# zhaoruiyang98/eftpipe

Measured on AMD Instinct MI355X. Metric: theory P_l(k) evaluations/sec (single tracer, Nk=512, l=0,2,4), higher is better.
Workload: dtype f64

## Files before the change

### eftpipe_amd/csrc/eftb_kernels.hpp

```cpp
#pragma once
#include <hip/hip_runtime.h>
#include <stdint.h>
#include <stdlib.h>

namespace eftb {

constexpr int NS = 80;
constexpr int NPOW = 257;
constexpr int NHALF = 128;
constexpr int NCH = 129;

constexpr int NROW = 24;

typedef double v4d __attribute__((ext_vector_type(4)));
typedef double v2d __attribute__((ext_vector_type(2)));

__device__ __forceinline__ void xcd_decode(int ntile, int& tile, int& group) {
    const int flat = blockIdx.x, ng = gridDim.x / ntile;
    if ((ng & 7) == 0) {
        const int slot = flat >> 3;
        tile = slot % ntile;
        group = (flat & 7) + 8 * (slot / ntile);
    } else {
        tile = flat % ntile;
// ... 1650 lines not shown
    double h[2];
#pragma unroll
    for (int v = 0; v < 2; ++v) h[v] = H[((size_t)v * NS + s0) * Nk + kc];
    double z = k2 * ct[42], y = k2 * ct[43];
    double b0, b1;
    powers(z * (1.0 / RS_ZS), b0, b1);
#pragma unroll
    for (int tau = 0; tau < NT; ++tau)
#pragma unroll
        for (int t = 0; t < 2; ++t) asm volatile("" : "+v"(aop[tau][t]));
    for (int s = s0; s < s1; ++s) {
        const int sn = s + 1 < s1 ? s + 1 : s;
        const double* ctn = RSC + ((size_t)w * NS + sn) * RS_REC;
        double cv[14 * NT];
#pragma unroll
        for (int i = 0; i < 14 * NT; ++i) cv[i] = ct[i];
        const double xn = ctn[42], yn0 = ctn[43];
        double hn[2];
#pragma unroll
        for (int v = 0; v < 2; ++v) hn[v] = H[((size_t)v * NS + sn) * Nk + kc];
        __builtin_amdgcn_sched_barrier(0);
        v4d D[NT];
#pragma unroll
        for (int tau = 0; tau < NT; ++tau) D[tau] = __builtin_amdgcn_mfma_f64_16x16x4f64(aop[tau][0], b0, (v4d){0.0, 0.0, 0.0, 0.0}, 0, 0, 0);
#pragma unroll
        for (int tau = 0; tau < NT; ++tau) D[tau] = __builtin_amdgcn_mfma_f64_16x16x4f64(aop[tau][1], b1, D[tau], 0, 0, 0);
        __builtin_amdgcn_sched_barrier(0);
        const double zn = k2 * xn, yn = k2 * yn0;
        double bn0, bn1;
        powers(zn * (1.0 / RS_ZS), bn0, bn1);
        const double zh[2] = {z * h[0], z * h[1]}, yh[2] = {y * h[0], y * h[1]};
#pragma unroll
        for (int tau = 0; tau < NT; ++tau) {
            const double W = fma(zh[tau], D[tau][0], fma(yh[0], D[tau][1], yh[1] * D[tau][2]));
            acc11[tau] = fma(W, cv[tau * 14], acc11[tau]);
            accCt[tau] = fma(W, cv[tau * 14 + 1], accCt[tau]);
#pragma unroll
            for (int i = 0; i < 12; ++i) accL[i] = fma(W, cv[tau * 14 + 2 + i], accL[i]);
        }
        __builtin_amdgcn_sched_barrier(0);
        ct = ctn;
        z = zn;
        y = yn;
        b0 = bn0;
        b1 = bn1;
        h[0] = hn[0];
        h[1] = hn[1];
    }
    if (!live) return;
    const int l = jg & 1;
    double o18[18], oA[3];
#pragma unroll
    for (int i = 0; i < 6; ++i) o18[i] = lct[i] * accCt[0] + lct[6 + i] * accCt[1];
#pragma unroll
    for (int i = 0; i < 12; ++i) o18[6 + i] = accL[i];
#pragma unroll
    for (int i = 0; i < 3; ++i) oA[i] = l11[i] * acc11[0] + l11[3 + i] * acc11[1];
    if (nsplit == 1) {
        double* dst = T + (((size_t)w * NL + l) * NROW) * Nk + k;
        if (jg < 2) {
#pragma unroll
            for (int i = 0; i < 18; ++i) dst[(size_t)(3 + i) * Nk] += o18[i];
        } else {
#pragma unroll
            for (int i = 0; i < 3; ++i) dst[(size_t)i * Nk] += oA[i];
        }
    } else {
        double* pw = part + (((size_t)w * nsplit + split) * NL + l) * 21 * Nk + k;
        if (jg < 2) {
#pragma unroll
            for (int i = 0; i < 18; ++i) pw[(size_t)(3 + i) * Nk] = o18[i];
        } else {
#pragma unroll
            for (int i = 0; i < 3; ++i) pw[(size_t)i * Nk] = oA[i];
        }
    }
}

__global__ __launch_bounds__(256) void resum_sum_kernel(int Nk, int Nl, int nchunk, const double* __restrict__ part,
                                                        double* __restrict__ T) {
    const int k = blockIdx.x * blockDim.x + threadIdx.x;
    const int i = blockIdx.y % 21, l = blockIdx.y / 21, w = blockIdx.z;
    if (k >= Nk) return;
    double a = 0.0;
    for (int c = 0; c < nchunk; ++c) a += part[((((size_t)w * nchunk + c) * Nl + l) * 21 + i) * Nk + k];
    T[(((size_t)w * Nl + l) * NROW + i) * Nk + k] += a;
}

constexpr int SPL_HB = 32;

constexpr int SPL_W = 128, SPL_LD = SPL_W + 2;

__global__ __launch_bounds__(256) __attribute__((amdgpu_num_vgpr(88))) void spline_kernel(int Nk, int nseries, int rlo, int rsel, const double* __restrict__ T, const double* __restrict__ band,
                                                     double* __restrict__ S) {
    __shared__ double ys[16 * SPL_LD];
    const int tid = threadIdx.x, lane = tid & 63, wave = tid >> 6, r = lane & 15, g = lane >> 4;
    int ktile, share;
    xcd_decode((Nk + 63) / 64, ktile, share);
    const int nshare = gridDim.x / ((Nk + 63) / 64);
    const int w0 = ktile * 64 - SPL_HB;
    const int it0 = ktile * 64 + 16 * wave;
    double bf[20];
#pragma unroll
    for (int t = 0; t < 20; ++t) {
        const int d = 4 * t + g - r, i = it0 + r;
        bf[t] = (d >= 0 && d <= 2 * SPL_HB && i < Nk) ? band[(size_t)d * Nk + i] : 0.0;
    }
    const int ngroups = (nseries + 15) / 16;
    const int per = (ngroups + nshare - 1) / nshare;
    const int g0 = share * per, g1 = min(ngroups, g0 + per);
    auto row_of = [&](int sp) { return rsel == NROW ? sp : (sp / rsel) * NROW + rlo + sp % rsel; };
    double pre[8];
    auto fetch = [&](int grp) {
#pragma unroll
        for (int u = 0; u < 8; ++u) {
            const int e = tid + 256 * u, sr = e >> 7, jj = w0 + (e & 127), series = grp * 16 + sr;
            pre[u] = (series < nseries && jj >= 0 && jj < Nk) ? T[(size_t)row_of(series) * Nk + jj] : 0.0;
        }
    };
    if (g0 < g1) fetch(g0);
    for (int grp = g0; grp < g1; ++grp) {
        __syncthreads();
#pragma unroll
        for (int u = 0; u < 8; ++u) {
            const int e = tid + 256 * u;
            ys[(e >> 7) * SPL_LD + (e & 127)] = pre[u];
        }
        __syncthreads();
        if (grp + 1 < g1) fetch(grp + 1);
        v4d acc = (v4d){0.0, 0.0, 0.0, 0.0};
        const double* yr = ys + r * SPL_LD + 16 * wave + g;
#pragma unroll
        for (int t = 0; t < 20; ++t) acc = __builtin_amdgcn_mfma_f64_16x16x4f64(yr[4 * t], bf[t], acc, 0, 0, 0);
        const int i = it0 + r;
#pragma unroll
        for (int q = 0; q < 4; ++q) {
            const int sr = g + 4 * q, series = grp * 16 + sr;
            if (series < nseries && i < Nk) S[(size_t)row_of(series) * Nk + i] = acc[q];
        }
    }
}

__device__ __forceinline__ int bspl_first(int i, int Nk) { return min(max(i - 1, 0), Nk - 4); }

__device__ inline int knot_interval(const double* __restrict__ kk, int Nk, double x) {
    int lo = 0, hi = Nk - 1;
    while (hi - lo > 1) {
        const int mid = (lo + hi) >> 1;
        if (kk[mid] <= x) lo = mid; else hi = mid;
    }
    return lo;
}

template <int NL>
__global__ __launch_bounds__(320) void ap_prefix_kernel(int nmu, const double* __restrict__ DAw, const double* __restrict__ Hw,
                                                        const double* __restrict__ fid, const double* __restrict__ mu,
                                                        const double* __restrict__ wmu, const double* __restrict__ legmu,
                                                        double* __restrict__ PS, double* __restrict__ ROOT) {
    constexpr int NS = NL * NL * 4, NCH = 8;
    extern __shared__ double sm[];
    double* s_rho = sm;
    double* s_lp = sm + nmu;
    double* s_wl = sm + (1 + NL) * nmu;
    double* s_tot = sm + (1 + 2 * NL) * nmu;
    const int w = blockIdx.x;
    const double qperp = DAw[w] / fid[0], qpar = fid[1] / Hw[w];
    const double F = qpar / qperp, g = 1.0 / (F * F) - 1.0;
    for (int j = threadIdx.x; j < nmu; j += blockDim.x) {
        const double m = mu[j];
        const double root = sqrt(1.0 + m * m * g);
        const double mp = m / (F * root), x2 = mp * mp;
        ROOT[(size_t)w * nmu + j] = root;
        s_rho[j] = g * m * m / (1.0 + root);
        s_lp[j] = 1.0;
        s_lp[nmu + j] = 0.5 * (3.0 * x2 - 1.0);
        if (NL > 2) s_lp[2 * nmu + j] = (35.0 * x2 * x2 - 30.0 * x2 + 3.0) * 0.125;
#pragma unroll
        for (int l = 0; l < NL; ++l) s_wl[l * nmu + j] = wmu[j] * legmu[l * nmu + j];
    }
    __syncthreads();
    const int seq = threadIdx.x % NS, ch = threadIdx.x / NS;
    const int q = seq & 3, l = (seq >> 2) % NL, lp = seq / (4 * NL);
    const int clen = (nmu + NCH - 1) / NCH, j0 = ch * clen, j1 = min(nmu, j0 + clen);
    double* ps = PS + (size_t)w * (nmu + 1) * NS + seq;
    auto term = [&](int j) {
        const double r = s_rho[j];
        const double rq = q == 0 ? 1.0 : (q == 1 ? r : (q == 2 ? r * r : r * r * r));
        return s_wl[l * nmu + j] * s_lp[lp * nmu + j] * rq;
    };
    if (ch < NCH) {
        double s = 0.0;
        for (int j = j0; j < j1; ++j) s += term(j);
        s_tot[seq * NCH + ch] = s;
    }
    __syncthreads();
    if (threadIdx.x < NS) {
        double run = 0.0;
        for (int c = 0; c < NCH; ++c) {
            const double t = s_tot[threadIdx.x * NCH + c];
            s_tot[threadIdx.x * NCH + c] = run;
            run += t;
        }
        PS[(size_t)w * (nmu + 1) * NS + threadIdx.x] = 0.0;
    }
    __syncthreads();
    if (ch < NCH) {
        double s = s_tot[seq * NCH + ch];
        for (int j = j0; j < j1; ++j) {
            s += term(j);
            ps[(size_t)(j + 1) * NS] = s;
        }
    }
}

template <int NL, bool BSPL>
__global__ __launch_bounds__(64) void ap_direct_kernel(int Nk, int nmu, int rlo, int nr, const double* __restrict__ kk, const double* __restrict__ DAw,
                                                       const double* __restrict__ Hw, const double* __restrict__ fid,
                                                       const double* __restrict__ mu, const double* __restrict__ wmu,
                                                       const double* __restrict__ legmu, const double* __restrict__ ROOT,
                                                       const double* __restrict__ T, const double* __restrict__ S, double* __restrict__ Tout,
                                                       const int4* __restrict__ META, const double* __restrict__ bias, double* __restrict__ Plk,
                                                       double* __restrict__ PlkHost, int msplit, int* __restrict__ nonfinite,
                                                       const double* __restrict__ LOCAL) {
    const int KT = (Nk + 63) / 64;
    int kt, w;
    xcd_decode(KT, kt, w);
    if (META && !META[(size_t)w * 2 * KT + 2 * kt + (threadIdx.x >> 5)].w) return;
    const int k = kt * 64 + threadIdx.x;
    if (k >= Nk) return;
    const double qperp = DAw[w] / fid[0], qpar = fid[1] / Hw[w], F = qpar / qperp;
    const double kq = kk[k] / qperp, c = 2.0 / (qperp * qperp * qpar);
    const double* root = ROOT + (size_t)w * nmu;
    const int i_first = knot_interval(kk, Nk, kq * root[0]);
    double ch0[NL], ch1[NL];
#pragma unroll
    for (int l = 0; l < NL; ++l) ch0[l] = ch1[l] = 0.0;
    const double* bw = bias ? bias + (size_t)w * NROW : nullptr;
    for (int r = 0; r < NROW; ++r) {
        const double br = bw ? bw[r] : 0.0;
        if (r >= nr || r < rlo) {
#pragma unroll
            for (int l = 0; l < NL; ++l) {
                const size_t o = (((size_t)w * NL + l) * NROW + r) * Nk + k;
                const double v = T[o];
                Tout[o] = v;
                if (r < msplit) ch0[l] = fma(br, v, ch0[l]); else ch1[l] = fma(br, v, ch1[l]);
            }
            continue;
        }
        const size_t rbase = ((size_t)w * NL * NROW + r) * Nk;
        double acc[NL];
#pragma unroll
        for (int l = 0; l < NL; ++l) acc[l] = 0.0;
        int i = i_first;
        for (int j = 0; j < nmu; ++j) {
            const double rt = root[j], kp = kq * rt;
            while (i < Nk - 2 && kk[i + 1] <= kp) ++i;
            while (i > 0 && kk[i] > kp) --i;
            const double klo = kk[i], h = kk[i + 1] - klo, ih = 1.0 / h, t = kp - klo;
            const double m = mu[j], mp = m / (F * rt), x2 = mp * mp;
            const double lpv[3] = {1.0, 0.5 * (3.0 * x2 - 1.0), (35.0 * x2 * x2 - 30.0 * x2 + 3.0) * 0.125};
            double P = 0.0;
            if (BSPL) {
                const double4* lc = reinterpret_cast<const double4*>(LOCAL + (size_t)i * 16);
                double be[4];
#pragma unroll
                for (int e = 0; e < 4; ++e) {
                    const double4 n4 = lc[e];
                    be[e] = fma(fma(fma(n4.w, t, n4.z), t, n4.y), t, n4.x);
                }
                const int J = bspl_first(i, Nk);
#pragma unroll
                for (int lp = 0; lp < NL; ++lp) {
                    const double* cp = S + rbase + (size_t)lp * NROW * Nk + J;
                    P = fma(fma(be[0], cp[0], fma(be[1], cp[1], fma(be[2], cp[2], be[3] * cp[3]))), lpv[lp], P);
                }
            } else {
#pragma unroll
                for (int lp = 0; lp < NL; ++lp) {
                    const size_t o = rbase + (size_t)lp * NROW * Nk + i;
                    const double ya = T[o], yb = T[o + 1], sa = S[o], sb = S[o + 1];
                    const double sl = (yb - ya) * ih;
                    const double c3 = (sa + sb - 2.0 * sl) * ih * ih;
                    const double c2 = (sl - sa) * ih - c3 * h;
                    P = fma(fma(fma(fma(c3, t, c2), t, sa), t, ya), lpv[lp], P);
                }
            }
            const double wj = wmu[j] * P;
#pragma unroll
            for (int l = 0; l < NL; ++l) acc[l] = fma(wj, legmu[(size_t)l * nmu + j], acc[l]);
        }
#pragma unroll
        for (int l = 0; l < NL; ++l) {
            const double v = c * acc[l];
            Tout[(((size_t)w * NL + l) * NROW + r) * Nk + k] = v;
            if (r < msplit) ch0[l] = fma(br, v, ch0[l]); else ch1[l] = fma(br, v, ch1[l]);
        }
    }
    if (bias) {
#pragma unroll
        for (int l = 0; l < NL; ++l) {
            const double a = ch0[l] + ch1[l];
            Plk[((size_t)w * NL + l) * Nk + k] = a;
            if (PlkHost) PlkHost[((size_t)w * NL + l) * Nk + k] = a;
            if (nonfinite && !(fabs(a) <= 1.79769313486231570815e308)) atomicMax(nonfinite, w + 1);
        }
// ... 474 lines not shown
    if (j0 < j1) {
        if (big) walk(std::true_type{});
        else walk(std::false_type{});
    }
    if (wave > 0) {
#pragma unroll
        for (int l = 0; l < NL; ++l) s_red[((size_t)(wave - 1) * NL + l) * 64 + lane] = acc[l];
    }
    __syncthreads();
    if (wave > 0 || k >= Nk) return;
    const double* bw = bias + (size_t)w * NROW;
#pragma unroll
    for (int l = 0; l < NL; ++l) {
        double a = acc[l];
#pragma unroll
        for (int q = 0; q < 3; ++q) a += s_red[((size_t)q * NL + l) * 64 + lane];
        double tot = cnorm * a;
        for (int r = direct0; r < NROW; ++r) tot = fma(bw[r], stoch_template(l, r - (NROW - 3), kk[k]), tot);
        Plk[((size_t)w * NL + l) * Nk + k] = tot;
        if (PlkHost) PlkHost[((size_t)w * NL + l) * Nk + k] = tot;
        if (nonfinite && !(fabs(tot) <= 1.79769313486231570815e308)) atomicMax(nonfinite, w + 1);
    }
}

template <int NL>
__global__ __launch_bounds__(256) void ap_plk_mom_kernel(int Nk, int nmu, const double* __restrict__ kk, const double* __restrict__ DAw,
                                                         const double* __restrict__ Hw, const double* __restrict__ fid, const double* __restrict__ mu,
                                                         const double* __restrict__ PS, const double* __restrict__ ROOT, const double* __restrict__ C,
                                                         const double* __restrict__ LOCAL, const double* __restrict__ T, const double* __restrict__ bias,
                                                         double* __restrict__ Plk, double* __restrict__ PlkHost, int* __restrict__ nonfinite, int direct0) {
    constexpr int NSQ = NL * NL * 4;
    extern __shared__ double sm[];
    double* s_k = sm;
    double* s_root = sm + Nk;
    double* red = sm + Nk + nmu;
    const int lane = threadIdx.x & 63, wave = threadIdx.x >> 6;
    const int KT = (Nk + 63) / 64;
    int kt, w;
    xcd_decode(KT, kt, w);
    const int k = kt * 64 + lane;
    for (int e = threadIdx.x; e < Nk; e += 256) s_k[e] = kk[e];
    for (int e = threadIdx.x; e < nmu; e += 256) s_root[e] = ROOT[(size_t)w * nmu + e];
    __syncthreads();
    const double qperp = DAw[w] / fid[0], qpar = fid[1] / Hw[w];
    const double F = qpar / qperp, g = 1.0 / (F * F) - 1.0;
    const bool live = k < Nk;
    const double kq = s_k[live ? k : Nk - 1] / qperp;
    const double inv_kq = 1.0 / kq, inv_g = 1.0 / g;
    const double* ps = PS + (size_t)w * (nmu + 1) * NSQ;
    const double* cw = C + (size_t)w * NL * NROW * Nk;
    const bool up = g > 0.0;
    const int dir = up ? 1 : -1;
    const double jscale = (nmu - 1) / mu[nmu - 1];
    double acc[NL];
#pragma unroll
    for (int l = 0; l < NL; ++l) acc[l] = 0.0;
    auto cross = [&](double kb) -> int {
        const double rc = kb * inv_kq, x = (rc * rc - 1.0) * inv_g;
        int j = nmu;
        if (x >= 0.0 && x < 1.0) j = (int)(sqrt(x) * jscale) + 1;
        j = max(0, min(j, nmu));
        while (j > 0 && (up ? kq * s_root[j - 1] >= kb : kq * s_root[j - 1] < kb)) --j;
        while (j < nmu && !(up ? kq * s_root[j] >= kb : kq * s_root[j] < kb)) ++j;
        return j;
    };
    const int i_first = knot_interval(s_k, Nk, kq * s_root[0]);
    const int i_last = knot_interval(s_k, Nk, kq * s_root[nmu - 1]);
    const int nslot = live ? (up ? i_last - i_first : i_first - i_last) + 1 : 0;
    for (int s = wave; s < nslot; s += 4) {
        const int i = i_first + s * dir;
        const double klo = s_k[i], khi = s_k[i + 1];
        const int ja = s == 0 ? 0 : cross(up ? klo : khi);
        const int jb = s == nslot - 1 ? nmu : cross(up ? khi : klo);
        if (jb <= ja) continue;
        const double* pa = ps + (size_t)ja * NSQ;
        const double* pb = ps + (size_t)jb * NSQ;
        double4 a4[NL][NL], b4[NL][NL];
#pragma unroll
        for (int lp = 0; lp < NL; ++lp)
#pragma unroll
            for (int l = 0; l < NL; ++l) {
                b4[lp][l] = *reinterpret_cast<const double4*>(pb + (lp * NL + l) * 4);
                a4[lp][l] = *reinterpret_cast<const double4*>(pa + (lp * NL + l) * 4);
            }
        const double4* lc = reinterpret_cast<const double4*>(LOCAL + (size_t)i * 16);
        const double4 e0 = lc[0], e1 = lc[1], e2 = lc[2], e3 = lc[3];
        const int J = bspl_first(i, Nk);
        double cc[NL][4];
#pragma unroll
        for (int lp = 0; lp < NL; ++lp) {
            const double* cp = cw + (size_t)lp * NROW * Nk + J;
            cc[lp][0] = cp[0]; cc[lp][1] = cp[1]; cc[lp][2] = cp[2]; cc[lp][3] = cp[3];
        }
        const double dl = kq - klo, dl2 = dl * dl, a2 = kq * kq;
        const double c10 = dl, c11 = kq, c20 = dl2, c21 = 2.0 * kq * dl, c22 = a2;
        const double c30 = dl2 * dl, c31 = 3.0 * kq * dl2, c32 = 3.0 * a2 * dl, c33 = a2 * kq;
#pragma unroll
        for (int lp = 0; lp < NL; ++lp) {
            const double p0 = fma(e0.x, cc[lp][0], fma(e1.x, cc[lp][1], fma(e2.x, cc[lp][2], e3.x * cc[lp][3])));
            const double p1 = fma(e0.y, cc[lp][0], fma(e1.y, cc[lp][1], fma(e2.y, cc[lp][2], e3.y * cc[lp][3])));
            const double p2 = fma(e0.z, cc[lp][0], fma(e1.z, cc[lp][1], fma(e2.z, cc[lp][2], e3.z * cc[lp][3])));
            const double p3 = fma(e0.w, cc[lp][0], fma(e1.w, cc[lp][1], fma(e2.w, cc[lp][2], e3.w * cc[lp][3])));
#pragma unroll
            for (int l = 0; l < NL; ++l) {
                const double d0 = b4[lp][l].x - a4[lp][l].x, d1 = b4[lp][l].y - a4[lp][l].y;
                const double d2 = b4[lp][l].z - a4[lp][l].z, d3 = b4[lp][l].w - a4[lp][l].w;
                const double m1 = fma(c10, d0, c11 * d1);
                const double m2 = fma(c20, d0, fma(c21, d1, c22 * d2));
                const double m3 = fma(c30, d0, fma(c31, d1, fma(c32, d2, c33 * d3)));
                acc[l] = fma(d0, p0, fma(m1, p1, fma(m2, p2, fma(m3, p3, acc[l]))));
            }
        }
    }
    if (wave > 0) {
#pragma unroll
        for (int l = 0; l < NL; ++l) red[((size_t)(wave - 1) * NL + l) * 64 + lane] = acc[l];
    }
    __syncthreads();
    if (wave > 0 || !live) return;
    const double cnorm = 2.0 / (qperp * qperp * qpar);
    const double* bw = bias + (size_t)w * NROW;
#pragma unroll
    for (int l = 0; l < NL; ++l) {
        double a = acc[l];
#pragma unroll
        for (int q = 0; q < 3; ++q) a += red[((size_t)q * NL + l) * 64 + lane];
        double tot = cnorm * a;
        for (int r = direct0; r < NROW; ++r) tot = fma(bw[r], stoch_template(l, r - (NROW - 3), kk[k]), tot);
        Plk[((size_t)w * NL + l) * Nk + k] = tot;
        if (PlkHost) PlkHost[((size_t)w * NL + l) * Nk + k] = tot;
        if (nonfinite && !(fabs(tot) <= 1.79769313486231570815e308)) atomicMax(nonfinite, w + 1);
    }
}

template <int NL, int NW>
__global__ __launch_bounds__(64 * NW) void ap_plk_fused_kernel(int Nk, int nmu, const double* __restrict__ kk, const double* __restrict__ DAw,
                                                           const double* __restrict__ Hw, const double* __restrict__ fid, const double* __restrict__ mu,
                                                           const double* __restrict__ wmu, const double* __restrict__ legmu, const double* __restrict__ C,
                                                           const double* __restrict__ LOCAL, const double* __restrict__ T, const double* __restrict__ bias,
                                                           double* __restrict__ Plk, double* __restrict__ PlkHost, int* __restrict__ nonfinite, int direct0) {
    constexpr int NSQ = NL * NL * 4, NT = 64 * NW, NCHK = NT / NSQ;
    extern __shared__ double sm[];
    double* s_k = sm;
    double* s_root = s_k + ((Nk + 1) & ~1);
    double* s_rho = s_root + nmu;
    double* s_lp = s_rho + nmu;
    double* s_wl = s_lp + NL * nmu;
    double* s_tot = s_wl + NL * nmu;
    double* s_ps = s_tot + NSQ * (NCHK + 1);
    double* s_pp = s_ps + (size_t)(nmu + 1) * NSQ;
    const int lane = threadIdx.x & 63, wave = threadIdx.x >> 6;
    constexpr int SPLIT = NW == 8 ? 1 : 2;
    const int half = blockIdx.x % SPLIT, w = blockIdx.x / SPLIT;
    const double qperp = DAw[w] / fid[0], qpar = fid[1] / Hw[w];
    const double F = qpar / qperp, g = 1.0 / (F * F) - 1.0;
    for (int e = threadIdx.x; e < Nk; e += NT) s_k[e] = kk[e];
    for (int j = threadIdx.x; j < nmu; j += NT) {
        const double m = mu[j];
        const double root = sqrt(1.0 + m * m * g);
        const double mp = m / (F * root), x2 = mp * mp, wj = wmu[j];
        s_root[j] = root;
        s_rho[j] = g * m * m / (1.0 + root);
        s_lp[j] = 1.0;
        s_lp[nmu + j] = 0.5 * (3.0 * x2 - 1.0);
        if (NL > 2) s_lp[2 * nmu + j] = (35.0 * x2 * x2 - 30.0 * x2 + 3.0) * 0.125;
#pragma unroll
        for (int l = 0; l < NL; ++l) s_wl[l * nmu + j] = wj * legmu[(size_t)l * nmu + j];
    }
    const double* cw = C + (size_t)w * NL * NROW * Nk;
    for (int i = threadIdx.x; i < Nk - 1; i += NT) {
        const int J = bspl_first(i, Nk);
        const double4* lc = reinterpret_cast<const double4*>(LOCAL + (size_t)i * 16);
        const double4 e0 = lc[0], e1 = lc[1], e2 = lc[2], e3 = lc[3];
        double cc[NL][4];
#pragma unroll
        for (int lp = 0; lp < NL; ++lp) {
            const double* cp = cw + (size_t)lp * NROW * Nk + J;
            cc[lp][0] = cp[0]; cc[lp][1] = cp[1]; cc[lp][2] = cp[2]; cc[lp][3] = cp[3];
        }
#pragma unroll
        for (int lp = 0; lp < NL; ++lp) {
            const double c0 = cc[lp][0], c1 = cc[lp][1], c2 = cc[lp][2], c3 = cc[lp][3];
            double4 pp;
            pp.x = fma(e0.x, c0, fma(e1.x, c1, fma(e2.x, c2, e3.x * c3)));
            pp.y = fma(e0.y, c0, fma(e1.y, c1, fma(e2.y, c2, e3.y * c3)));
            pp.z = fma(e0.z, c0, fma(e1.z, c1, fma(e2.z, c2, e3.z * c3)));
            pp.w = fma(e0.w, c0, fma(e1.w, c1, fma(e2.w, c2, e3.w * c3)));
            *reinterpret_cast<double4*>(s_pp + ((size_t)i * NL + lp) * 4) = pp;
        }
    }
    __syncthreads();
    {
        constexpr int CL = NW == 8 ? 16 : 32;
        const int seq = threadIdx.x % NSQ, ch = threadIdx.x / NSQ;
        const int q = seq & 3, l = (seq >> 2) % NL, lp = seq / (4 * NL);
        const int clen = (nmu + NCHK - 1) / NCHK, j0 = ch * clen, nj = ch < NCHK ? max(0, min(nmu - j0, clen)) : 0;
        double v[CL];
#pragma unroll
        for (int u = 0; u < CL; ++u) {
            const int j = min(j0 + u, nmu - 1);
            const double r = s_rho[j];
            const double rq = q == 0 ? 1.0 : (q == 1 ? r : (q == 2 ? r * r : r * r * r));
            v[u] = u < nj ? s_wl[l * nmu + j] * s_lp[lp * nmu + j] * rq : 0.0;
        }
#pragma unroll
        for (int u = 1; u < CL; ++u) v[u] += v[u - 1];
        if (ch < NCHK) s_tot[seq * (NCHK + 1) + ch] = v[CL - 1];
        __syncthreads();
        if (threadIdx.x < NSQ) {
            double run = 0.0;
            for (int c = 0; c < NCHK; ++c) {
                const double t = s_tot[threadIdx.x * (NCHK + 1) + c];
                s_tot[threadIdx.x * (NCHK + 1) + c] = run;
                run += t;
            }
            s_ps[threadIdx.x] = 0.0;
        }
        __syncthreads();
        if (ch < NCHK) {
            const double off = s_tot[seq * (NCHK + 1) + ch];
#pragma unroll
            for (int u = 0; u < CL; ++u)
                if (u < nj) s_ps[(size_t)(j0 + u + 1) * NSQ + seq] = off + v[u];
        }
    }
    __syncthreads();
    const int KT = (Nk + 63) / 64;
    const bool up = g > 0.0;
    const int dir = up ? 1 : -1;
    const double inv_g = 1.0 / g, jscale = (nmu - 1) / mu[nmu - 1];
    const double cnorm = 2.0 / (qperp * qperp * qpar);
    const double* bw = bias + (size_t)w * NROW;
    for (int kt = SPLIT * wave + half; kt < KT; kt += SPLIT * NW) {
        const int k = kt * 64 + lane;
        const bool live = k < Nk;
        const double kq = s_k[live ? k : Nk - 1] / qperp, inv_kq = 1.0 / kq;
        double tst[NL][3];
#pragma unroll
        for (int l = 0; l < NL; ++l)
#pragma unroll
            for (int r = 0; r < 3; ++r) tst[l][r] = live && NROW - 3 + r >= direct0 ? stoch_template(l, r, s_k[k]) : 0.0;
        auto cross = [&](double kb) -> int {
            const double rc = kb * inv_kq, x = (rc * rc - 1.0) * inv_g;
            int j = nmu;
            if (x >= 0.0 && x < 1.0) j = (int)(sqrt(x) * jscale) + 1;
            j = max(0, min(j, nmu));
            while (j > 0 && (up ? kq * s_root[j - 1] >= kb : kq * s_root[j - 1] < kb)) --j;
            while (j < nmu && !(up ? kq * s_root[j] >= kb : kq * s_root[j] < kb)) ++j;
            return j;
        };
        const int i_first = knot_interval(s_k, Nk, kq * s_root[0]);
        const int i_last = knot_interval(s_k, Nk, kq * s_root[nmu - 1]);
        const int nslot = live ? (up ? i_last - i_first : i_first - i_last) + 1 : 0;
        double acc[NL];
#pragma unroll
        for (int l = 0; l < NL; ++l) acc[l] = 0.0;
        int ja = 0;
        for (int s = 0; s < nslot; ++s) {
            const int i = i_first + s * dir;
            const double klo = s_k[i], khi = s_k[i + 1];
            const int jb = s == nslot - 1 ? nmu : cross(up ? khi : klo);
            if (jb > ja) {
                const double dl = kq - klo, kq2 = kq * kq;
                const double* pa = s_ps + (size_t)ja * NSQ;
                const double* pb = s_ps + (size_t)jb * NSQ;
                const double* pi = s_pp + (size_t)i * NL * 4;
#pragma unroll
                for (int lp = 0; lp < NL; ++lp) {
                    const double4 p = *reinterpret_cast<const double4*>(pi + lp * 4);
                    const double w0 = fma(fma(fma(p.w, dl, p.z), dl, p.y), dl, p.x);
                    const double w1 = kq * fma(fma(3.0 * p.w, dl, 2.0 * p.z), dl, p.y);
                    const double w2 = kq2 * fma(3.0 * p.w, dl, p.z);
                    const double w3 = kq2 * kq * p.w;
#pragma unroll
                    for (int l = 0; l < NL; ++l) {
                        const double4 b4 = *reinterpret_cast<const double4*>(pb + (lp * NL + l) * 4);
                        const double4 a4 = *reinterpret_cast<const double4*>(pa + (lp * NL + l) * 4);
                        acc[l] = fma(b4.x - a4.x, w0, fma(b4.y - a4.y, w1, fma(b4.z - a4.z, w2, fma(b4.w - a4.w, w3, acc[l]))));
                    }
                }
                ja = jb;
            }
        }
        if (!live) continue;
#pragma unroll
        for (int l = 0; l < NL; ++l) {
            double tot = cnorm * acc[l];
#pragma unroll
            for (int r = 0; r < 3; ++r)
                if (NROW - 3 + r >= direct0) tot = fma(bw[NROW - 3 + r], tst[l][r], tot);
            Plk[((size_t)w * NL + l) * Nk + k] = tot;
            if (PlkHost) PlkHost[((size_t)w * NL + l) * Nk + k] = tot;
            if (nonfinite && !(fabs(tot) <= 1.79769313486231570815e308)) atomicMax(nonfinite, w + 1);
        }
    }
}

__global__ __launch_bounds__(256) void stage_copy_kernel(const double* __restrict__ src, double* __restrict__ dst, size_t n) {
    for (size_t i = (size_t)blockIdx.x * blockDim.x + threadIdx.x; i < n; i += (size_t)gridDim.x * blockDim.x) dst[i] = src[i];
}

struct StageSeg { const double* src; double* dst; unsigned n, first; };
struct StageSegs { StageSeg s[48]; int n; };
__global__ __launch_bounds__(256) void stage_gather_kernel(StageSegs sg) {
    const unsigned i = blockIdx.x * 256u + threadIdx.x;
    int seg = 0;
    for (int q = 1; q < sg.n; ++q)
        if (i >= sg.s[q].first) seg = q;
    const StageSeg g = sg.s[seg];
    const unsigned j = i - g.first;
    if (j < g.n) g.dst[j] = g.src[j];
}

__global__ void wake_kernel() {}

__global__ __launch_bounds__(256) void copy16_kernel(const double* __restrict__ src, double* __restrict__ dst, size_t n) {
    const size_t n2 = n / 2;
    const double2* s2 = reinterpret_cast<const double2*>(src);
    double2* d2 = reinterpret_cast<double2*>(dst);
    for (size_t i = (size_t)blockIdx.x * blockDim.x + threadIdx.x; i < n2; i += (size_t)gridDim.x * blockDim.x) d2[i] = s2[i];
    if ((n & 1) && blockIdx.x == 0 && threadIdx.x == 0) dst[n - 1] = src[n - 1];
}

__global__ __launch_bounds__(256) void copy8_kernel(const double* __restrict__ src, double* __restrict__ dst, size_t n) {
    for (size_t i = (size_t)blockIdx.x * blockDim.x + threadIdx.x; i < n; i += (size_t)gridDim.x * blockDim.x) dst[i] = src[i];
}

__global__ __launch_bounds__(256) void reduce_kernel(int Nx, int Nl, int msplit, const double* __restrict__ bias, const double* __restrict__ T,
                                                     double* __restrict__ Plk, double* __restrict__ PlkHost, int* __restrict__ nonfinite) {
    const int k = blockIdx.x * blockDim.x + threadIdx.x, l = blockIdx.y, w = blockIdx.z;
    if (k >= Nx) return;
    const double* b = bias + (size_t)w * NROW;
    const double* t = T + (((size_t)w * Nl + l) * NROW) * Nx + k;
    double a0 = 0.0, a1 = 0.0;
    for (int r = 0; r < msplit; ++r) a0 = fma(b[r], t[(size_t)r * Nx], a0);
    for (int r = msplit; r < NROW; ++r) a1 = fma(b[r], t[(size_t)r * Nx], a1);
    const double a = a0 + a1;
    Plk[((size_t)w * Nl + l) * Nx + k] = a;
    if (PlkHost) PlkHost[((size_t)w * Nl + l) * Nx + k] = a;
    if (nonfinite && !(fabs(a) <= 1.79769313486231570815e308)) atomicMax(nonfinite, w + 1);
}

__global__ __launch_bounds__(256) void reduce_nnlo_kernel(int Nx, int Nl, const double* __restrict__ biasn, const double* __restrict__ TN,
                                                          double* __restrict__ Plk, int* __restrict__ nonfinite) {
    const int k = blockIdx.x * blockDim.x + threadIdx.x, l = blockIdx.y, w = blockIdx.z;
    if (k >= Nx) return;
    const double* b = biasn + (size_t)w * 3;
    const double* t = TN + (((size_t)w * Nl + l) * NROW + 3) * Nx + k;
    const double a = Plk[((size_t)w * Nl + l) * Nx + k] + (b[0] * t[0] + b[1] * t[(size_t)Nx] + b[2] * t[(size_t)2 * Nx]);
    Plk[((size_t)w * Nl + l) * Nx + k] = a;
    if (nonfinite && !(fabs(a) <= 1.79769313486231570815e308)) atomicMax(nonfinite, w + 1);
}

constexpr int MARG_MAXG = 24, MARG_NG1 = MARG_MAXG + 1, MARG_OUT = 2 + MARG_MAXG;

__global__ __launch_bounds__(256) void marg_build_kernel(int nl, int nx, int ntr, int ndata, int nG, const int* __restrict__ index,
                                                         const double* __restrict__ data, const double* __restrict__ rows,
                                                         const double* __restrict__ T, const double* __restrict__ rowsn,
                                                         const double* __restrict__ TN, double* __restrict__ Vout) {
    extern __shared__ double sm[];
    const int ng1 = nG + 1, w = blockIdx.x, tid = threadIdx.x;
    double* R = sm;
    double* V = Vout + (size_t)w * ng1 * ndata;
    for (int e = tid; e < ntr * ng1 * NROW; e += 256)
        R[e] = rows[((size_t)w * ntr + e / (ng1 * NROW)) * MARG_NG1 * NROW + e % (ng1 * NROW)];
    __syncthreads();
    for (int a = tid; a < ndata; a += 256) {
        const int l = index[a] / nx, x = index[a] % nx, tr = l / nl;
        const double* t = T + ((size_t)w * ntr * nl + l) * NROW * nx + x;
        const double* Rt = R + tr * ng1 * NROW;
        double tv[NROW];
#pragma unroll
        for (int r = 0; r < NROW; ++r) tv[r] = t[(size_t)r * nx];
        for (int g = 0; g < ng1; ++g) {
            double s0 = 0.0, s1 = 0.0;
#pragma unroll
            for (int r = 0; r < NROW; r += 2) {
                s0 = fma(Rt[g * NROW + r], tv[r], s0);
                s1 = fma(Rt[g * NROW + r + 1], tv[r + 1], s1);
            }
            if (TN) {
                const double* tn = TN + (((size_t)w * ntr * nl + l) * NROW + 3) * nx + x;
                const double* rn = rowsn + (((size_t)w * ntr + tr) * MARG_NG1 + g) * 3;
                s0 += rn[0] * tn[0] + rn[1] * tn[(size_t)nx] + rn[2] * tn[(size_t)2 * nx];
            }
            V[(size_t)g * ndata + a] = s0 + s1 - (g == 0 ? data[a] : 0.0);
        }
    }
}

__global__ __launch_bounds__(256) void marg_solve_kernel(int ndata, int nG, int jeffreys, const double* __restrict__ mu,
                                                         const double* __restrict__ sinv, const double* __restrict__ Vall,
                                                         const double* __restrict__ Uall, double* __restrict__ out) {
    __shared__ double G[MARG_NG1 * MARG_NG1];
    __shared__ double A[MARG_MAXG][MARG_MAXG + 1];
    __shared__ double mrow[MARG_MAXG];
    __shared__ int s_piv, s_sign;
    __shared__ double s_logdet;
    const int ng1 = nG + 1, w = blockIdx.x, tid = threadIdx.x;
    const double* V = Vall + (size_t)w * ng1 * ndata;
    const double* U = Uall + (size_t)w * ng1 * ndata;
    const int sub = tid & 15, grp = tid >> 4;
    for (int e = grp; e < ng1 * ng1; e += 16) {
        const int i = e / ng1, j = e % ng1;
        double s0 = 0.0;
        for (int b = sub; b < ndata; b += 16) s0 = fma(V[(size_t)i * ndata + b], U[(size_t)j * ndata + b], s0);
        s0 += __shfl_xor(s0, 8, 16);
        s0 += __shfl_xor(s0, 4, 16);
        s0 += __shfl_xor(s0, 2, 16);
        s0 += __shfl_xor(s0, 1, 16);
        if (sub == 0) G[e] = s0;
    }
    __syncthreads();
    for (int e = tid; e < nG * nG; e += 256) {
        const int i = e / nG, j = e % nG;
        A[i][j] = 0.5 * (G[(i + 1) * ng1 + j + 1] + G[(j + 1) * ng1 + i + 1]) + (i == j ? sinv[i] : 0.0);
    }
    if (tid == 0) {
        s_sign = 1;
        s_logdet = 0.0;
    }
    __syncthreads();
    __shared__ int piv[MARG_MAXG];
    for (int c = 0; c < nG; ++c) {
        if (tid == 0) {
            int p = c;
            for (int i = c + 1; i < nG; ++i)
                if (fabs(A[i][c]) > fabs(A[p][c])) p = i;
            piv[c] = p;
            s_piv = p;
        }
        __syncthreads();
        const int p = s_piv;
        if (p != c && tid < nG) {
            const double t = A[c][tid];
            A[c][tid] = A[p][tid];
            A[p][tid] = t;
        }
        __syncthreads();
        const double dpiv = A[c][c];
        if (tid == 0) {
            if (p != c) s_sign = -s_sign;
            if (dpiv < 0.0) s_sign = -s_sign;
            if (dpiv == 0.0 || dpiv != dpiv) s_sign = 0;
            s_logdet += log(fabs(dpiv));
// ... 1629 lines not shown
```

Before: 1.906 million.

## Split per-k slot loop across paired waves and hoist prologue global loads

The per-k slot loop in the fused AP kernel is now split in half across two waves, which are paired so that one handles the tail of a tile and another the head. Partial sums are reduced through shared memory that reuses the s_rho region, so wave load is more balanced and the idle waves get work. Global loads of mu, weights, Legendre values, LOCAL, C and bias are issued at kernel start, before the qperp divisions, and the two knot binary searches are interleaved to expose ILP. The cost is extra __syncthreads, shared-memory reuse of the prefix scratch, and a changed summation order (fp contract off).

```diff
diff --git a/eftpipe_amd/csrc/eftb_kernels.hpp b/eftpipe_amd/csrc/eftb_kernels.hpp
--- a/eftpipe_amd/csrc/eftb_kernels.hpp
+++ b/eftpipe_amd/csrc/eftb_kernels.hpp
@@ -1826,6 +1826,18 @@
     return lo;
 }
 
+__device__ __forceinline__ void knot_interval2(const double* __restrict__ kk, int Nk, double x0, double x1, int& i0, int& i1) {
+    int lo0 = 0, hi0 = Nk - 1, lo1 = 0, hi1 = Nk - 1;
+    while (hi0 - lo0 > 1 || hi1 - lo1 > 1) {
+        const int mid0 = (lo0 + hi0) >> 1, mid1 = (lo1 + hi1) >> 1;
+        const double v0 = kk[mid0], v1 = kk[mid1];
+        if (hi0 - lo0 > 1) { if (v0 <= x0) lo0 = mid0; else hi0 = mid0; }
+        if (hi1 - lo1 > 1) { if (v1 <= x1) lo1 = mid1; else hi1 = mid1; }
+    }
+    i0 = lo0;
+    i1 = lo1;
+}
+
 template <int NL>
 __global__ __launch_bounds__(320) void ap_prefix_kernel(int nmu, const double* __restrict__ DAw, const double* __restrict__ Hw,
                                                         const double* __restrict__ fid, const double* __restrict__ mu,
@@ -2606,31 +2618,59 @@
     const int lane = threadIdx.x & 63, wave = threadIdx.x >> 6;
     constexpr int SPLIT = NW == 8 ? 1 : 2;
     const int half = blockIdx.x % SPLIT, w = blockIdx.x / SPLIT;
+    const double* cw = C + (size_t)w * NL * NROW * Nk;
+    const double* bw = bias + (size_t)w * NROW;
+    const int jt0 = min((int)threadIdx.x, nmu - 1), it0 = min((int)threadIdx.x, Nk - 2);
+    const double m0 = mu[jt0], wj0 = wmu[jt0], mu_last = mu[nmu - 1];
+    double lg0[NL];
+#pragma unroll
+    for (int l = 0; l < NL; ++l) lg0[l] = legmu[(size_t)l * nmu + jt0];
+    double4 e00, e01, e02, e03;
+    double cc0[NL][4];
+    {
+        const double4* lc = reinterpret_cast<const double4*>(LOCAL + (size_t)it0 * 16);
+        e00 = lc[0]; e01 = lc[1]; e02 = lc[2]; e03 = lc[3];
+        const int J = bspl_first(it0, Nk);
+#pragma unroll
+        for (int lp = 0; lp < NL; ++lp) {
+            const double* cp = cw + (size_t)lp * NROW * Nk + J;
+            cc0[lp][0] = cp[0]; cc0[lp][1] = cp[1]; cc0[lp][2] = cp[2]; cc0[lp][3] = cp[3];
+        }
+    }
+    double bwr[3];
+#pragma unroll
+    for (int r = 0; r < 3; ++r) bwr[r] = bw[NROW - 3 + r];
+    for (int e = threadIdx.x; e < Nk; e += NT) s_k[e] = kk[e];
     const double qperp = DAw[w] / fid[0], qpar = fid[1] / Hw[w];
     const double F = qpar / qperp, g = 1.0 / (F * F) - 1.0;
-    for (int e = threadIdx.x; e < Nk; e += NT) s_k[e] = kk[e];
-    for (int j = threadIdx.x; j < nmu; j += NT) {
-        const double m = mu[j];
+    if (threadIdx.x < nmu) {
+        const int j = threadIdx.x;
+        const double m = m0;
         const double root = sqrt(1.0 + m * m * g);
-        const double mp = m / (F * root), x2 = mp * mp, wj = wmu[j];
+        const double mp = m / (F * root), x2 = mp * mp, wj = wj0;
         s_root[j] = root;
         s_rho[j] = g * m * m / (1.0 + root);
         s_lp[j] = 1.0;
         s_lp[nmu + j] = 0.5 * (3.0 * x2 - 1.0);
         if (NL > 2) s_lp[2 * nmu + j] = (35.0 * x2 * x2 - 30.0 * x2 + 3.0) * 0.125;
 #pragma unroll
-        for (int l = 0; l < NL; ++l) s_wl[l * nmu + j] = wj * legmu[(size_t)l * nmu + j];
-    }
-    const double* cw = C + (size_t)w * NL * NROW * Nk;
+        for (int l = 0; l < NL; ++l) s_wl[l * nmu + j] = wj * lg0[l];
+    }
     for (int i = threadIdx.x; i < Nk - 1; i += NT) {
-        const int J = bspl_first(i, Nk);
-        const double4* lc = reinterpret_cast<const double4*>(LOCAL + (size_t)i * 16);
-        const double4 e0 = lc[0], e1 = lc[1], e2 = lc[2], e3 = lc[3];
+        const bool first = i == (int)threadIdx.x;
+        double4 e0 = e00, e1 = e01, e2 = e02, e3 = e03;
         double cc[NL][4];
 #pragma unroll
-        for (int lp = 0; lp < NL; ++lp) {
-            const double* cp = cw + (size_t)lp * NROW * Nk + J;
-            cc[lp][0] = cp[0]; cc[lp][1] = cp[1]; cc[lp][2] = cp[2]; cc[lp][3] = cp[3];
+        for (int lp = 0; lp < NL; ++lp) { cc[lp][0] = cc0[lp][0]; cc[lp][1] = cc0[lp][1]; cc[lp][2] = cc0[lp][2]; cc[lp][3] = cc0[lp][3]; }
+        if (!first) {
+            const int J = bspl_first(i, Nk);
+            const double4* lc = reinterpret_cast<const double4*>(LOCAL + (size_t)i * 16);
+            e0 = lc[0]; e1 = lc[1]; e2 = lc[2]; e3 = lc[3];
+#pragma unroll
+            for (int lp = 0; lp < NL; ++lp) {
+                const double* cp = cw + (size_t)lp * NROW * Nk + J;
+                cc[lp][0] = cp[0]; cc[lp][1] = cp[1]; cc[lp][2] = cp[2]; cc[lp][3] = cp[3];
+            }
         }
 #pragma unroll
         for (int lp = 0; lp < NL; ++lp) {
@@ -2682,69 +2722,91 @@
     const int KT = (Nk + 63) / 64;
     const bool up = g > 0.0;
     const int dir = up ? 1 : -1;
-    const double inv_g = 1.0 / g, jscale = (nmu - 1) / mu[nmu - 1];
+    const double inv_g = 1.0 / g, jscale = (nmu - 1) / mu_last;
     const double cnorm = 2.0 / (qperp * qperp * qpar);
-    const double* bw = bias + (size_t)w * NROW;
-    for (int kt = SPLIT * wave + half; kt < KT; kt += SPLIT * NW) {
-        const int k = kt * 64 + lane;
-        const bool live = k < Nk;
-        const double kq = s_k[live ? k : Nk - 1] / qperp, inv_kq = 1.0 / kq;
-        double tst[NL][3];
-#pragma unroll
-        for (int l = 0; l < NL; ++l)
-#pragma unroll
-            for (int r = 0; r < 3; ++r) tst[l][r] = live && NROW - 3 + r >= direct0 ? stoch_template(l, r, s_k[k]) : 0.0;
-        auto cross = [&](double kb) -> int {
-            const double rc = kb * inv_kq, x = (rc * rc - 1.0) * inv_g;
-            int j = nmu;
-            if (x >= 0.0 && x < 1.0) j = (int)(sqrt(x) * jscale) + 1;
-            j = max(0, min(j, nmu));
-            while (j > 0 && (up ? kq * s_root[j - 1] >= kb : kq * s_root[j - 1] < kb)) --j;
-            while (j < nmu && !(up ? kq * s_root[j] >= kb : kq * s_root[j] < kb)) ++j;
-            return j;
-        };
-        const int i_first = knot_interval(s_k, Nk, kq * s_root[0]);
-        const int i_last = knot_interval(s_k, Nk, kq * s_root[nmu - 1]);
-        const int nslot = live ? (up ? i_last - i_first : i_first - i_last) + 1 : 0;
-        double acc[NL];
-#pragma unroll
-        for (int l = 0; l < NL; ++l) acc[l] = 0.0;
-        int ja = 0;
-        for (int s = 0; s < nslot; ++s) {
-            const int i = i_first + s * dir;
-            const double klo = s_k[i], khi = s_k[i + 1];
-            const int jb = s == nslot - 1 ? nmu : cross(up ? khi : klo);
-            if (jb > ja) {
-                const double dl = kq - klo, kq2 = kq * kq;
-                const double* pa = s_ps + (size_t)ja * NSQ;
-                const double* pb = s_ps + (size_t)jb * NSQ;
-                const double* pi = s_pp + (size_t)i * NL * 4;
-#pragma unroll
-                for (int lp = 0; lp < NL; ++lp) {
-                    const double4 p = *reinterpret_cast<const double4*>(pi + lp * 4);
-                    const double w0 = fma(fma(fma(p.w, dl, p.z), dl, p.y), dl, p.x);
-                    const double w1 = kq * fma(fma(3.0 * p.w, dl, 2.0 * p.z), dl, p.y);
-                    const double w2 = kq2 * fma(3.0 * p.w, dl, p.z);
-                    const double w3 = kq2 * kq * p.w;
-#pragma unroll
-                    for (int l = 0; l < NL; ++l) {
-                        const double4 b4 = *reinterpret_cast<const double4*>(pb + (lp * NL + l) * 4);
-                        const double4 a4 = *reinterpret_cast<const double4*>(pa + (lp * NL + l) * 4);
-                        acc[l] = fma(b4.x - a4.x, w0, fma(b4.y - a4.y, w1, fma(b4.z - a4.z, w2, fma(b4.w - a4.w, w3, acc[l]))));
+    const int nT = (KT - half + SPLIT - 1) / SPLIT;
+    double* const red = s_rho;
+    const int R = min(NW, (nmu * (1 + 2 * NL) + NSQ * (NCHK + 1)) / (NL * 64));
+    for (int j0 = 0; j0 < nT; j0 += R) {
+        const int nr = min(nT - j0, R);
+        if (j0 > 0) __syncthreads();
+        double acc1[NL];
+        int k1 = 0;
+        bool live1 = false;
+        for (int u = 0; u < 2 && wave < nr; ++u) {
+            const int jt = u == 0 ? j0 + nr - 1 - wave : j0 + wave;
+            const int k = (SPLIT * jt + half) * 64 + lane;
+            const bool live = k < Nk;
+            const double kq = s_k[live ? k : Nk - 1] / qperp, inv_kq = 1.0 / kq;
+            auto cross = [&](double kb) -> int {
+                const double rc = kb * inv_kq, x = (rc * rc - 1.0) * inv_g;
+                int j = nmu;
+                if (x >= 0.0 && x < 1.0) j = (int)(sqrt(x) * jscale) + 1;
+                j = max(0, min(j, nmu));
+                while (j > 0 && (up ? kq * s_root[j - 1] >= kb : kq * s_root[j - 1] < kb)) --j;
+                while (j < nmu && !(up ? kq * s_root[j] >= kb : kq * s_root[j] < kb)) ++j;
+                return j;
+            };
+            int i_first, i_last;
+            knot_interval2(s_k, Nk, kq * s_root[0], kq * s_root[nmu - 1], i_first, i_last);
+            const int nslot = live ? (up ? i_last - i_first : i_first - i_last) + 1 : 0;
+            const int h = (nslot + 1) >> 1, s1 = u == 0 ? nslot : h;
+            int s = u == 0 ? h : 0;
+            double acc[NL];
+#pragma unroll
+            for (int l = 0; l < NL; ++l) acc[l] = 0.0;
+            int ja = 0;
+            if (u == 0 && s < s1) {
+                const int i = i_first + (s - 1) * dir;
+                ja = cross(up ? s_k[i + 1] : s_k[i]);
+            }
+            for (; s < s1; ++s) {
+                const int i = i_first + s * dir;
+                const double klo = s_k[i], khi = s_k[i + 1];
+                const int jb = s == nslot - 1 ? nmu : cross(up ? khi : klo);
+                if (jb > ja) {
+                    const double dl = kq - klo, kq2 = kq * kq;
+                    const double* qa = s_ps + (size_t)ja * NSQ;
+                    const double* qb = s_ps + (size_t)jb * NSQ;
+                    const double* pi = s_pp + (size_t)i * NL * 4;
+#pragma unroll
+                    for (int lp = 0; lp < NL; ++lp) {
+                        const double4 p = *reinterpret_cast<const double4*>(pi + lp * 4);
+                        const double w0 = fma(fma(fma(p.w, dl, p.z), dl, p.y), dl, p.x);
+                        const double w1 = kq * fma(fma(3.0 * p.w, dl, 2.0 * p.z), dl, p.y);
+                        const double w2 = kq2 * fma(3.0 * p.w, dl, p.z);
+                        const double w3 = kq2 * kq * p.w;
+#pragma unroll
+                        for (int l = 0; l < NL; ++l) {
+                            const double4 b4 = *reinterpret_cast<const double4*>(qb + (lp * NL + l) * 4);
+                            const double4 a4 = *reinterpret_cast<const double4*>(qa + (lp * NL + l) * 4);
+                            acc[l] = fma(b4.x - a4.x, w0, fma(b4.y - a4.y, w1, fma(b4.z - a4.z, w2, fma(b4.w - a4.w, w3, acc[l]))));
+                        }
                     }
+                    ja = jb;
                 }
-                ja = jb;
-            }
-        }
-        if (!live) continue;
+            }
+            if (u == 0) {
+#pragma unroll
+                for (int l = 0; l < NL; ++l) red[((nr - 1 - wave) * NL + l) * 64 + lane] = acc[l];
+            } else {
+#pragma unroll
+                for (int l = 0; l < NL; ++l) acc1[l] = acc[l];
+                k1 = k;
+                live1 = live;
+            }
+        }
+        __syncthreads();
+        if (!live1) continue;
 #pragma unroll
         for (int l = 0; l < NL; ++l) {
-            double tot = cnorm * acc[l];
+#pragma clang fp contract(off)
+            double tot = cnorm * (acc1[l] + red[(wave * NL + l) * 64 + lane]);
 #pragma unroll
             for (int r = 0; r < 3; ++r)
-                if (NROW - 3 + r >= direct0) tot = fma(bw[NROW - 3 + r], tst[l][r], tot);
-            Plk[((size_t)w * NL + l) * Nk + k] = tot;
-            if (PlkHost) PlkHost[((size_t)w * NL + l) * Nk + k] = tot;
+                if (NROW - 3 + r >= direct0) tot = fma(bwr[r], stoch_template(l, r, s_k[k1]), tot);
+            Plk[((size_t)w * NL + l) * Nk + k1] = tot;
+            if (PlkHost) PlkHost[((size_t)w * NL + l) * Nk + k1] = tot;
             if (nonfinite && !(fabs(tot) <= 1.79769313486231570815e308)) atomicMax(nonfinite, w + 1);
         }
     }
```

Result: slower. 1.851 million (-2.9%).
